# cgranerob/Land-Surface-Temperature-Super-Resolution-with-a-Scale-Invariance-Free-Neural-Approach

Measured on AMD Instinct MI355X. Metric: LST+NDVI 256x256 patches/sec (train fwd+bwd), whole job, higher is better.
Workload: dtype f32; 1 GPU; ModelB SIF-NN-SR2 (gradFTM loss) batch 64/GPU, synthetic 256x256, 1x MI355X, fwd+loss+bwd+Adam; batch_per_gpu=64, patch=256x256 (LST 64x64 + NDVI 256x256), parallelism=dp1, loss=sr2

## Files before the change

include/sifsr_hip.h:

```cpp
#ifndef SIFSR_HIP_H
#define SIFSR_HIP_H
#include <stddef.h>

#ifdef __cplusplus
#define SIFSR_API extern "C" __attribute__((visibility("default")))
#else
#define SIFSR_API
#endif

SIFSR_API int sifsr_abi_version(void);
SIFSR_API int sifsr_num_params(void);
SIFSR_API int sifsr_num_running(void);
SIFSR_API int sifsr_layer_table(int* out, int capacity_rows);

SIFSR_API size_t sifsr_model_workspace_bytes(int B, int H, int W, int training);
SIFSR_API int sifsr_model_workspace_regions(int B, int H, int W, size_t* out, int capacity);
SIFSR_API int sifsr_model_forward(const float* x, float* sr, const float* params, float* running, long long* nbt,
                                  void* workspace, size_t workspace_bytes, int B, int H, int W, int training,
                                  float momentum, float eps, void* stream);
SIFSR_API int sifsr_model_backward(const float* x, const float* dsr, const float* params, float* grads,
                                   void* workspace, size_t workspace_bytes, int B, int H, int W, void* stream);
SIFSR_API int sifsr_model_forward_ex(const float* x, float* sr, const float* params, float* running, long long* nbt,
                                     void* workspace, size_t workspace_bytes, int B, int H, int W, int training,
                                     float momentum, float eps, int compute, void* stream);
SIFSR_API int sifsr_model_backward_ex(const float* x, const float* dsr, const float* params, float* grads, void* workspace,
                                      size_t workspace_bytes, int B, int H, int W, int compute, void* stream);

SIFSR_API int sifsr_pack_conv_weights(const float* w_oihw, int cin, int cout, float* wfwd, float* wdgrad, void* stream);
SIFSR_API int sifsr_conv3x3_stat_blocks(int B, int H, int W, int cout);
SIFSR_API int sifsr_conv3x3_fwd(const float* src0, int C0, const float* scale0, const float* shift0,
                                const float* src1, int C1, const float* scale1, const float* shift1,
                                const float* wfwd, float* y, int cout, float* stat_partials, int B, int H, int W,
                                void* stream);
SIFSR_API int sifsr_conv3x3_dgrad(const float* dy, int cout, const float* wdgrad, const float* w_oihw, int cin,
                                  float* g0, int C0, float* g1, int C1, const float* addend, int B, int H, int W,
                                  void* stream);
SIFSR_API int sifsr_conv3x3_dgrad_fused(const float* g, const float* y, const float* coef_f, int cout, const float* wdgrad,
                                        const float* wwd, int cin, float* g0, int C0, float* g1, int C1, const float* addend,
                                        float* border, int B, int H, int W, void* stream);
SIFSR_API int sifsr_pack_conv_weights_wino(const float* w_oihw, int cin, int cout, float* wwf, float* wwd, void* stream);
SIFSR_API int sifsr_conv3x3_stat_blocks_wino(int B, int H, int W, int cin, int cout);
SIFSR_API int sifsr_conv3x3_fwd_wino(const float* src0, int C0, const float* scale0, const float* shift0,
                                     const float* src1, int C1, const float* scale1, const float* shift1,
                                     const float* wfwd, const float* wwf, float* y, int cout, float* stat_partials,
                                     int B, int H, int W, void* stream);
SIFSR_API int sifsr_conv3x3_dgrad_wino(const float* dy, int cout, const float* wdgrad, const float* wwd, int cin,
                                       float* g0, int C0, float* g1, int C1, const float* addend, int B, int H, int W,
                                       void* stream);
SIFSR_API int sifsr_conv3x3_fwd_bf16(const float* src0, int C0, const float* scale0, const float* shift0, const float* src1,
                                     int C1, const float* scale1, const float* shift1, const float* wdgrad, float* y,
                                     int cout, float* stat_partials, int B, int H, int W, void* stream);
SIFSR_API int sifsr_conv3x3_dgrad_bf16(const float* dy, int cout, const float* wdgrad, int cin, float* g0, int C0, float* g1,
                                       int C1, const float* addend, int B, int H, int W, void* stream);
SIFSR_API size_t sifsr_conv3x3_wgrad_scratch_floats(int cin, int cout, int nblk);
SIFSR_API int sifsr_conv3x3_wgrad(const float* src0, int C0, const float* scale0, const float* shift0,
                                  const float* src1, int C1, const float* scale1, const float* shift1,
                                  const float* dy, int cout, float* scratch, int nblk, float* dw, int B, int H, int W,
                                  void* stream);
SIFSR_API int sifsr_conv3x3_wgrad_fused(const float* src0, int C0, const float* scale0, const float* shift0,
                                        const float* src1, int C1, const float* scale1, const float* shift1,
                                        const float* g, const float* y, const float* coef_f, int cout, float* scratch,
                                        int nblk, float* dw, int B, int H, int W, void* stream);
// ... 118 lines not shown
```

land-surface-temperature-super-resolution-with-a-scale-invariance-free-neural-approach_amd/csrc/capi.hip:

```cpp
#include "../../include/sifsr_hip.h"

#include "engine.h"

#define S(stream) ((hipStream_t)(stream))

static ConvSrc mk_src(const float* p, int C, const float* sc, const float* sh) {
  ConvSrc s; s.ptr = p; s.scale = p ? sc : nullptr; s.shift = p ? sh : nullptr; s.C = p ? C : 0; s.coff = 0; s.nq = p ? C / 16 : 0;
  return s;
}

int sifsr_abi_version(void) { return 3; }
int sifsr_num_params(void) { return sifsr_net().total_params; }
int sifsr_num_running(void) { return sifsr_net().total_running; }
int sifsr_layer_table(int* out, int capacity_rows) {
  const NetTable& nt = sifsr_net();
  for (int l = 0; l < SIFSR_NUM_BN_LAYERS && l < capacity_rows; ++l) {
    const LayerInfo& L = nt.L[l];
    int* r = out + 8 * l;
    r[0] = L.cin; r[1] = L.cout; r[2] = L.level; r[3] = L.w_off; r[4] = L.gamma_off; r[5] = L.beta_off; r[6] = L.run_off; r[7] = L.ch_off;
  }
  return SIFSR_NUM_BN_LAYERS;
}

size_t sifsr_model_workspace_bytes(int B, int H, int W, int training) {
// ... 114 lines not shown
  int rc = launch_conv3x3_mfma(a, cin, 1, S(stream));
  if (rc) return rc;
  return launch_dgrad_border_fix(dy, cout, wdgrad, cin, g0, C0, C0, g1 ? g1 : g0, g1 ? C1 : C0, B, H, W, S(stream));
}

int sifsr_conv3x3_dgrad_fused(const float* g, const float* y, const float* coef_f, int cout, const float* wdgrad,
                              const float* wwd, int cin, float* g0, int C0, float* g1, int C1, const float* addend, float* border,
                              int B, int H, int W, void* stream) {
  if (cout % 16 || cin % 16 || C0 % 16 || (g1 && (C1 % 16 || C0 + C1 != cin)) || (!g1 && C0 != cin) || (addend && g1))
    return SIFSR_ERR_SHAPE;
  if (!g || !y || !coef_f || !border) return SIFSR_ERR_ARG;
  ConvArgs a;
  a.src[0] = mk_src(g, cout, nullptr, nullptr); a.src[1] = mk_src(nullptr, 0, nullptr, nullptr);
  a.bw_y = y; a.bw_coef = coef_f; a.bw_border = border;
  a.dst[0].ptr = g0; a.dst[0].C = C0; a.dst[0].coff = 0;
  a.dst[1].ptr = g1 ? g1 : g0; a.dst[1].C = g1 ? C1 : C0; a.dst[1].coff = 0;
  a.wpack = wdgrad; a.wpack_wino = wwd; a.addend = addend; a.addC = cin; a.stat_partials = nullptr; a.dst_split = C0 / 16;
  a.B = B; a.H = H; a.W = W; a.NQ = cout / 16;
  int rc = launch_conv3x3_mfma(a, cin, 1, S(stream));
  if (rc) return rc;
  return launch_dgrad_border_fix(border, cout, wdgrad, cin, g0, C0, C0, g1 ? g1 : g0, g1 ? C1 : C0, B, H, W, S(stream));
}

static int conv3x3_fwd_lowp(int mode, const float* src0, int C0, const float* scale0, const float* shift0, const float* src1, int C1,
                            const float* scale1, const float* shift1, const float* wdgrad, float* y, int cout,
                            float* stat_partials, int B, int H, int W, void* stream) {
  if (!src0 || !wdgrad || C0 % 16 || (src1 && C1 % 16)) return SIFSR_ERR_SHAPE;
  ConvArgs a;
  a.src[0] = mk_src(src0, C0, scale0, shift0);
  a.src[1] = mk_src(src1, C1, scale1, shift1);
  a.dst[0].ptr = y; a.dst[0].C = cout; a.dst[0].coff = 0; a.dst[1] = a.dst[0];
  a.NQ = a.src[0].nq + a.src[1].nq;
  const size_t n = (size_t)9 * (16 * a.NQ) * cout;
  a.wpack = wdgrad + n; a.bf16 = mode;
  a.addend = nullptr; a.addC = 0; a.stat_partials = stat_partials; a.dst_split = cout / 16;
  a.B = B; a.H = H; a.W = W;
  return launch_conv3x3_mfma(a, cout, 0, S(stream));
}
int sifsr_conv3x3_fwd_bf16(const float* src0, int C0, const float* scale0, const float* shift0, const float* src1, int C1,
                           const float* scale1, const float* shift1, const float* wdgrad, float* y, int cout,
                           float* stat_partials, int B, int H, int W, void* stream) {
  return conv3x3_fwd_lowp(1, src0, C0, scale0, shift0, src1, C1, scale1, shift1, wdgrad, y, cout, stat_partials, B, H, W, stream);
}
static int conv3x3_dgrad_lowp(int mode, const float* dy, int cout, const float* wdgrad, int cin, float* g0, int C0, float* g1, int C1,
                              const float* addend, int B, int H, int W, void* stream) {
  if (cout % 16 || cin % 16 || C0 % 16 || (g1 && (C1 % 16 || C0 + C1 != cin)) || (!g1 && C0 != cin) || (addend && g1))
// ... 372 lines not shown
```

land-surface-temperature-super-resolution-with-a-scale-invariance-free-neural-approach_amd/csrc/conv.h:

```cpp
#pragma once
#include "common.h"
#include "diag.h"

struct ConvSrc {
  const float* ptr;
  const float* scale;
  const float* shift;
  int C;
  int coff;
  int nq;
};

struct ConvDst {
  float* ptr;
  int C;
  int coff;
};

struct ConvArgs {
  ConvSrc src[2];
  ConvDst dst[2];
  const float* wpack;
  const float* wpack_wino = nullptr;
  const float* addend;
  float* stat_partials;
  int addC;
  int dst_split;
  int B, H, W;
  int NQ;
  int bf16 = 0;
  const float* bn_y = nullptr;
  const float* bn_scale = nullptr;
  const float* bn_shift = nullptr;
  const float* bw_y = nullptr;
  const float* bw_coef = nullptr;
  float* bw_border = nullptr;
};

int launch_conv3x3_mfma(const ConvArgs& a, int cout, int zero_pad, hipStream_t s);
bool conv3x3_use_wino(const ConvArgs& a, int cout);
bool conv3x3_wino8_applies(int nb, int nq);
int launch_conv3x3_wino8(const ConvArgs& a, int nb, int zero_pad, bool dyf, int grid, int ntiles, int lgx, int lgy, hipStream_t s);
int conv3x3_wino_kind(const ConvArgs& a, int cout, int zero_pad);
int conv3x3_grid_blocks(int B, int H, int W, int cout, int wino = 0);

struct WgradArgs {
  ConvSrc src[2];
  const float* dy;
  float* slabs;
  int B, H, W;
  int NQ;
  int ntiles;
  int bf16 = 0;
  const float* dy_y = nullptr;
  const float* dy_coef = nullptr;
};
int launch_conv3x3_wgrad(const WgradArgs& a, int cin, int cout, int nblk, hipStream_t s);
int wgrad_nbi_chunk(const WgradArgs& a, int cin);
int launch_wgrad_reduce(const float* slabs, int nblk, int cin, int cout, int nbi_chunk, float* dw_oihw, hipStream_t s);
size_t wgrad_slab_floats(int cin, int cout);
struct WgradReduceJob { size_t slab_off; int nblk, cin, cout, nbi_chunk, w_off; };
int launch_wgrad_reduce_batched(const float* ws, const WgradReduceJob* jobs, int njobs, float* grads, hipStream_t s);

bool conv3x3_wgrad_use_wino(const WgradArgs& a, int cin, int cout);
int wgrad_wino_nbi_chunk(int cin);
int launch_conv3x3_wgrad_wino(const WgradArgs& a, int cin, int cout, int nblk, hipStream_t s);
template <typename V4, typename GET>
// ... 26 lines not shown
  float* dy_border = nullptr;
  const float* wpack_wino;
  float* gin;
  const float* addend = nullptr;
  const float* bn_y = nullptr;
  const float* bn_scale = nullptr;
  const float* bn_shift = nullptr;
  float* stat_partials = nullptr;
  float* slabs;
  int B, H, W;
  const float* pool_gp = nullptr;
  int store_dz = 0;
  int half = 0;
};
bool conv3x3_bwd16_applies(int B, int H, int W);
int conv3x3_bwd16_grid(int B, int H, int W);
int launch_conv3x3_bwd16(const Bwd16Args& a, hipStream_t s);

int launch_dgrad_border_fix(const float* dy, int Cout, const float* wdg_layer, int Cin, float* g0, int C0,
                            int split_ch, float* g1, int C1, int B, int H, int W, hipStream_t s, int bf16 = 0,
                            const float* bn_y = nullptr, const float* bn_scale = nullptr, const float* bn_shift = nullptr,
                            float* bn_partials = nullptr, int masked = 0);
int dgrad_border_waves(int B, int H, int W, int Cin);

int launch_pack_weights(const float* params, float* wfwd, float* wdgrad, hipStream_t s, float* wwf = nullptr, float* wwd = nullptr,
                        long long* nbt = nullptr, int nbt_n = 0);
```

land-surface-temperature-super-resolution-with-a-scale-invariance-free-neural-approach_amd/csrc/conv_mfma.hip:

```cpp
#include "conv.h"

#include "switches.h"

namespace {

constexpr int PW = 18;
constexpr int PLANE = 336;
constexpr int WPITCH = 20, WHALF = 10, WPLANE = 364;

typedef __attribute__((ext_vector_type(4))) unsigned u32x4;

static __device__ __forceinline__ __amdgpu_buffer_rsrc_t make_rsrc(const float* p, unsigned bytes) {
  return __builtin_amdgcn_make_buffer_rsrc(const_cast<float*>(p), 0, (int)bytes, 0x00020000);
}
static __device__ __forceinline__ float4 bload4(__amdgpu_buffer_rsrc_t r, unsigned voff, unsigned soff) {
  const u32x4 v = __builtin_amdgcn_raw_buffer_load_b128(r, (int)voff, (int)soff, 0);
  return make_float4(__uint_as_float(v.x), __uint_as_float(v.y), __uint_as_float(v.z), __uint_as_float(v.w));
}
static __device__ __forceinline__ void bstore4(__amdgpu_buffer_rsrc_t r, unsigned voff, unsigned soff, float4 v) {
  u32x4 u;
  u.x = __float_as_uint(v.x); u.y = __float_as_uint(v.y); u.z = __float_as_uint(v.z); u.w = __float_as_uint(v.w);
  __builtin_amdgcn_raw_buffer_store_b128(u, r, (int)voff, (int)soff, 0);
}
constexpr unsigned OOB = 0xFFFFFF00u;
// ... 752 lines not shown
    if (corner) {
#pragma unroll
      for (int sd = 0; sd < 2; ++sd) {
        const int xc = sd == 0 ? 0 : W - 1;
        const bool on = (sd == 0 ? cl : cr) && valid && qx == xc;
        rv[0] = dyload(poff(qy, xc, on), (unsigned)q * 64u);
        rv[1] = dyload(poff(yin, xc, on), (unsigned)q * 64u);
        wv[0] = ld4(wbase + ((size_t)q * 9 + (8 - (1 * 3 + 2 * sd))) * 256);
        wv[1] = ld4(wbase + ((size_t)q * 9 + (8 - ((ty_tb + 1) * 3 + 2 * sd))) * 256);
        if (bf16) { rv[0] = round_bf16x4(rv[0]); rv[1] = round_bf16x4(rv[1]); }
        mac(wv[0], rv[0], false);
        mac(wv[1], add4(rv[0], rv[1]), false);
      }
    }
  }
  if (valid && !masked) {
    float4 v = g_old;
    v.x += acc[0]; v.y += acc[1]; v.z += acc[2]; v.w += acc[3];
    if (bf16) stA4<true>(dbase, de, v); else stA4<false>(dbase, de, v);
  }
  if (bn_partials != nullptr) {
    float d1[4] = {0.f, 0.f, 0.f, 0.f}, d2[4] = {0.f, 0.f, 0.f, 0.f};
    if (valid) {
      const float4 yv = bf16 ? ldA4<true>(bn_y, pix_o * 16 + 4 * kq) : ldA4<false>(bn_y, pix_o * 16 + 4 * kq);
      const float4 bsc = ld4(bn_scale + 4 * kq), bsh = ld4(bn_shift + 4 * kq);
      const float yy[4] = {yv.x, yv.y, yv.z, yv.w}, scv[4] = {bsc.x, bsc.y, bsc.z, bsc.w}, shv[4] = {bsh.x, bsh.y, bsh.z, bsh.w};
#pragma unroll
      for (int r = 0; r < 4; ++r) {
        const float dz = fmaf(yy[r], scv[r], shv[r]) > 0.f ? acc[r] : 0.f;
        d1[r] = dz; d2[r] = dz * yy[r];
      }
      if (masked) {
        const float4 v = make_float4(g_old.x + d1[0], g_old.y + d1[1], g_old.z + d1[2], g_old.w + d1[3]);
        if (bf16) stA4<true>(dbase, de, v); else stA4<false>(dbase, de, v);
      }
    }
#pragma unroll
    for (int r = 0; r < 4; ++r)
#pragma unroll
      for (int m = 1; m < 16; m <<= 1) { d1[r] += __shfl_xor(d1[r], m); d2[r] += __shfl_xor(d2[r], m); }
    if (px == 0) {
#pragma unroll
      for (int r = 0; r < 4; ++r) {
        bn_partials[((size_t)wave_g * 16 + 4 * kq + r) * 2 + 0] = d1[r];
        bn_partials[((size_t)wave_g * 16 + 4 * kq + r) * 2 + 1] = d2[r];
      }
    }
  }
}

}

bool conv3x3_use_wino(const ConvArgs& a, int cout) {
  return !sifsr_switches().no_wino && a.wpack_wino != nullptr && a.bf16 == 0 && cout <= 64 && a.H % 2 == 0 && a.W % 2 == 0 && (cout > 16 || a.NQ <= 2);
}

int conv3x3_wino_kind(const ConvArgs& a, int cout, int zero_pad) {
  if (!conv3x3_use_wino(a, cout)) return 0;
  return (cout == 16 && !zero_pad) ? 2 : 1;
}

int conv3x3_grid_blocks(int B, int H, int W, int cout, int wino) {
  const int ntiles = B * ((H + 15) / 16) * ((W + 15) / 16);
  const int per_cu = wino ? (wino == 2 ? 2 : 1) : (cout >= 64 ? 1 : 2);
  const int gmax = 256 * per_cu;
  if (ntiles <= gmax) return ntiles;
  const int rounds = (ntiles + gmax - 1) / gmax;
  int g = (ntiles + rounds - 1) / rounds;
  g = (g + 7) & ~7;
  return g < ntiles ? g : ntiles;
}

int launch_conv3x3_mfma(const ConvArgs& a, int cout, int zero_pad, hipStream_t s) {
  if (a.H < 1 || a.W < 1 || cout % 16 || a.NQ < 1 || a.src[0].nq + a.src[1].nq != a.NQ) return SIFSR_ERR_SHAPE;
  if (a.bf16 < 0 || a.bf16 > 1) return SIFSR_ERR_ARG;
  if (!a.src[0].ptr || !a.dst[0].ptr || !a.wpack) return SIFSR_ERR_ARG;
  const int ntiles = a.B * ((a.H + 15) / 16) * ((a.W + 15) / 16);
  const dim3 grid(conv3x3_grid_blocks(a.B, a.H, a.W, cout)), block(512);
  const int nb = cout / 16;
  const size_t npix = (size_t)a.B * a.H * a.W;
  auto pow2 = [](int v) { return v > 0 && (v & (v - 1)) == 0; };
  auto lg = [](int v) { int l = 0; while ((1 << l) < v) ++l; return l; };
  int cmax = a.src[0].C > a.src[1].C ? a.src[0].C : a.src[1].C;
  cmax = cmax > a.dst[0].C ? cmax : a.dst[0].C;
  cmax = cmax > a.dst[1].C ? cmax : a.dst[1].C;
  if (npix * cmax * 4 >= ((size_t)1 << 32) - 4096) return SIFSR_ERR_SHAPE;
  if (!pow2(a.src[0].C) || (a.src[1].ptr && !pow2(a.src[1].C))) return SIFSR_ERR_SHAPE;
  const int tx_ = (a.W + 15) / 16, ty_ = (a.H + 15) / 16;
  const int lgx = (pow2(tx_) && pow2(ty_)) ? lg(tx_) : -1, lgy = lgx >= 0 ? lg(ty_) : -1;
  const bool dyf = a.bw_y != nullptr;
  if (dyf && (!zero_pad || !a.bw_coef || a.src[1].ptr || a.src[0].scale || a.src[0].coff)) return SIFSR_ERR_ARG;
  if (nb == 8 && conv3x3_use_wino(a, 64) && a.stat_partials == nullptr && a.dst_split % 4 == 0) {
    for (int h = 0; h < 2; ++h) {
      ConvArgs w = a;
      w.wpack_wino = a.wpack_wino + (size_t)h * 4 * a.NQ * 16 * 256;
      const bool first = 4 * h < a.dst_split;
      w.dst[0] = first ? a.dst[0] : a.dst[1];
      w.dst[0].coff += first ? 64 * h : 16 * (4 * h - a.dst_split);
      w.dst[1] = w.dst[0];
      w.dst_split = 4;
      if (a.addend != nullptr) w.addend = a.addend + 64 * h;
      const int rc = launch_conv3x3_mfma(w, 64, zero_pad, s);
      if (rc != SIFSR_OK) return rc;
    }
    return SIFSR_OK;
  }
  if (conv3x3_use_wino(a, cout)) {
    ConvArgs w = a;
    w.wpack = a.wpack_wino;
    const dim3 wgrid(conv3x3_grid_blocks(a.B, a.H, a.W, cout, conv3x3_wino_kind(a, cout, zero_pad)));
    if (conv3x3_wino8_applies(nb, a.NQ)) return launch_conv3x3_wino8(w, nb, zero_pad, dyf, (int)wgrid.x, ntiles, lgx, lgy, s);
#define SIFSR_WINO_LAUNCH(NBV, ZP, DY) hipLaunchKernelGGL((conv3x3_mfma_kernel<NBV, ZP, 0, DY, true>), wgrid, block, 0, s, w, ntiles, lgx, lgy)
#define SIFSR_WINO_CASE(NBV)                                                                              \
  case NBV:                                                                                               \
// ... 59 lines not shown
  SIFSR_LAUNCH_CHECK();
  return SIFSR_OK;
}

int launch_pack_weights_one(const float* w, int cin, int cout, float* wfwd, float* wdg, hipStream_t s, float* wwf, float* wwd) {
  PackTable tb;
  tb.w_off[0] = 0; tb.cin[0] = cin; tb.cout[0] = cout; tb.p_off[0] = 0;
  const int n = 9 * cin * cout;
  const dim3 grid((n + 255) / 256 > 64 ? 64 : (n + 255) / 256, 1);
  if (wfwd != nullptr && wdg != nullptr) {
    hipLaunchKernelGGL(pack_weights_kernel, grid, dim3(256), 0, s, w, wfwd, wdg, tb);
    SIFSR_LAUNCH_CHECK();
  }
  if (wwf != nullptr && wwd != nullptr) {
    hipLaunchKernelGGL(pack_wino_kernel, dim3(grid.x * 2, 1), dim3(256), 0, s, w, wwf, wwd, tb);
    SIFSR_LAUNCH_CHECK();
  }
  return SIFSR_OK;
}

int dgrad_border_waves(int B, int H, int W, int Cin) {
  return B * (2 * ((W + 15) / 16) + 2 * ((H - 2 + 15) / 16)) * (Cin / 16);
}

int launch_dgrad_border_fix(const float* dy, int Cout, const float* wdg_layer, int Cin, float* g0, int C0,
                            int split_ch, float* g1, int C1, int B, int H, int W, hipStream_t s, int bf16,
                            const float* bn_y, const float* bn_scale, const float* bn_shift, float* bn_partials, int masked) {
  if (bn_partials != nullptr && (Cin != 16 || !bn_y || !bn_scale || !bn_shift)) return SIFSR_ERR_ARG;
  if (masked && bn_partials == nullptr) return SIFSR_ERR_ARG;
  if (H < 3 || W < 2 || Cin % 16 || Cout % 16) return SIFSR_ERR_SHAPE;
  const int waves = B * (2 * ((W + 15) / 16) + 2 * ((H - 2 + 15) / 16)) * (Cin / 16);
  hipLaunchKernelGGL(dgrad_border_kernel, dim3((waves + 3) / 4), dim3(256), 0, s, dy, Cout, wdg_layer, Cin, g0, C0,
                     split_ch, g1, C1, B, H, W, bf16, bn_y, bn_scale, bn_shift, bn_partials, masked);
  SIFSR_LAUNCH_CHECK();
  return SIFSR_OK;
}
```

land-surface-temperature-super-resolution-with-a-scale-invariance-free-neural-approach_amd/csrc/conv_wino8.hip:

```cpp
#include "conv.h"
#include "switches.h"

SIFSR_DIAG_CLOCK_DECL
SIFSR_DIAG_CLOCK8_DECL
namespace {

constexpr int PW = 18;
constexpr int WPITCH = 20, WHALF = 10, WPLANE = 364;

typedef __attribute__((ext_vector_type(4))) unsigned u32x4;
static __device__ __forceinline__ __amdgpu_buffer_rsrc_t make_rsrc(const float* p, unsigned bytes) {
  return __builtin_amdgcn_make_buffer_rsrc(const_cast<float*>(p), 0, (int)bytes, 0x00020000);
}
static __device__ __forceinline__ float4 bload4(__amdgpu_buffer_rsrc_t r, unsigned voff, unsigned soff) {
  const u32x4 v = __builtin_amdgcn_raw_buffer_load_b128(r, (int)voff, (int)soff, 0);
  return make_float4(__uint_as_float(v.x), __uint_as_float(v.y), __uint_as_float(v.z), __uint_as_float(v.w));
}
static __device__ __forceinline__ void bstore4(__amdgpu_buffer_rsrc_t r, unsigned voff, unsigned soff, float4 v) {
  u32x4 u;
  u.x = __float_as_uint(v.x); u.y = __float_as_uint(v.y); u.z = __float_as_uint(v.z); u.w = __float_as_uint(v.w);
  __builtin_amdgcn_raw_buffer_store_b128(u, r, (int)voff, (int)soff, 0);
}
constexpr unsigned OOB = 0xFFFFFF00u;

template <int NB, bool ZERO_PAD, bool DYF>
__global__ __launch_bounds__(512, 2) void conv3x3_wino8_kernel(const ConvArgs a, const int ntiles, const int lgx, const int lgy) {
  static_assert(NB == 2 || NB == 4, "32 or 64 output channels");
  static_assert(!DYF || ZERO_PAD, "the fused BatchNorm backward belongs to the input-gradient pass");
  constexpr int NGRP = NB == 4 ? 2 : 1;

  __shared__ float4 lds[2][4 * WPLANE];
  __shared__ float red[8][16][2];
  __shared__ float4 coef[8][4][4];

  const int tid = threadIdx.x;
  const int lane = tid & 63;
  const int wave8 = __builtin_amdgcn_readfirstlane(tid >> 6);
  __builtin_amdgcn_s_setprio(2);
  const int H = a.H, W = a.W;
  const int tiles_x = (W + 15) / 16, tiles_y = (H + 15) / 16;
  const int NQ = a.NQ;
  const unsigned npix = (unsigned)a.B * (unsigned)H * (unsigned)W;

  const int G = gridDim.x;
  const bool xcd_map = (G % 8 == 0) && (ntiles % 8 == 0);
  const int t_lo = xcd_map ? (blockIdx.x % 8) * (ntiles / 8) : 0;
  const int t_hi = xcd_map ? t_lo + ntiles / 8 : ntiles;
  const int t_step = xcd_map ? G / 8 : G;
  int t = t_lo + (xcd_map ? blockIdx.x / 8 : blockIdx.x);
  auto tile_pos = [&](int tt, int& tb, int& txi, int& tyi) {
    if (lgx >= 0) { tyi = (tt >> lgx) & (tiles_y - 1); tb = tt >> (lgx + lgy); txi = (tt + tyi + tb) & (tiles_x - 1); }
    else { txi = tt % tiles_x; const int r = tt / tiles_x; tyi = r % tiles_y; tb = r / tiles_y; }
  };

  const __amdgpu_buffer_rsrc_t rs0 = make_rsrc(a.src[0].ptr, npix * a.src[0].C * 4u);
  const __amdgpu_buffer_rsrc_t rs1 = make_rsrc(a.src[1].ptr ? a.src[1].ptr : a.src[0].ptr, npix * (a.src[1].ptr ? a.src[1].C : a.src[0].C) * 4u);
// ... 51 lines not shown
    const int ch = (first ? a.src[0].coff + 16 * q : a.src[1].coff + 16 * (q - a.src[0].nq));
    const unsigned soff = ((unsigned)pix_base << lgc) + (unsigned)ch * 4u;
    const __amdgpu_buffer_rsrc_t r = first ? rs0 : rs1;
#pragma unroll
    for (int it = 0; it < 3; ++it) {
      const unsigned voff = (ZERO_PAD && pixv[it] < 0) ? OOB : (((unsigned)pixv[it] << lgc) + (unsigned)cg * 16u);
      stg[it] = bload4(r, voff, soff);
      if (DYF) sty[it] = bload4(rsy, voff, soff);
    }
    if (it_q + 1 < NQ) ++it_q;
    else if (it_t + t_step < t_hi) { it_t += t_step; it_q = 0; set_tile(it_t); }
  };
  if (tid < NQ * 16) {
    const int q = tid >> 4, kind = (tid >> 2) & 3, c4 = tid & 3;
    const bool first = q < a.src[0].nq;
    const int C = first ? a.src[0].C : a.src[1].C;
    const int ch = (first ? a.src[0].coff + 16 * q : a.src[1].coff + 16 * (q - a.src[0].nq));
    const float* scp = first ? a.src[0].scale : a.src[1].scale;
    const float* shp = first ? a.src[0].shift : a.src[1].shift;
    float4 v = make_float4(0.f, 0.f, 0.f, 0.f);
    if (DYF) v = ld4(a.bw_coef + kind * C + ch + 4 * c4);
    else if (scp != nullptr && kind < 2) v = ld4((kind ? shp : scp) + ch + 4 * c4);
    coef[q][kind][c4] = v;
  }
  auto write_stage = [&](float4* Lb) {
    const int q = stg_q, tS = stg_t;
    const bool first = q < a.src[0].nq;
    const bool praw = !DYF && (first ? a.src[0].scale : a.src[1].scale) == nullptr;
    const float4 psc = coef[q][0][cg], psh = coef[q][1][cg];
    float4 k1A = psc, k0A = psc;
    if (DYF) { k1A = coef[q][2][cg]; k0A = coef[q][3][cg]; }
    int wb = 0, wy0 = 0, wx0 = 0;
    bool winterior = true;
    if (DYF) {
      int txi, tyi;
      tile_pos(tS, wb, txi, tyi);
      wy0 = tyi * 16 - 1; wx0 = txi * 16 - 1;
      winterior = txi > 0 && tyi > 0 && txi + 1 < tiles_x && tyi + 1 < tiles_y;
    }
#pragma unroll
    for (int it = 0; it < 3; ++it) {
      float4 v = stg[it];
      const bool mine = it < 2 || st2;
      if (DYF) {
        v = bn_bwd4(v, sty[it], psc, psh, k1A, k0A);
        if (!winterior) {
// ... 130 lines not shown
        for (int b = 0; b < 4; ++b) Mc[b] = __builtin_amdgcn_mfma_f32_16x16x4f32(wr[b].w, dh[ar][b][1], Mc[b], 0, 0, 0);
        if (g == NGRP - 1) {
          __builtin_amdgcn_sched_barrier(0);
#pragma unroll
          for (int b = 0; b < 4; ++b) wq[4 * ar + b] = bload4(rww, (unsigned)lane * 16u, wsoff(qn, 4 * ar + b));
        }
        if (ar > 0) out_row(ar - 1, M[(ar - 1) & 1]);
      }
      out_row(3, M[1]);
      SIFSR_DIAG_T(g3_);
      SIFSR_DIAG_ADD(dt_rd, g1_ - g0_); SIFSR_DIAG_ADD(dt_tr, g2_ - g1_); SIFSR_DIAG_ADD(dt_mm, g3_ - g2_);
    }
    __builtin_amdgcn_s_setprio(3);
    SIFSR_DIAG_T(c2);

    if (!stage_first && more) {
      write_stage(lds[buf ^ 1]);
      issue_loads();
    }

    if (last_q) {
      int cb, txi, tyi;
      tile_pos(t, cb, txi, tyi);
      const bool do_stats = a.stat_partials != nullptr;
      const bool d0 = nb0 < a.dst_split;
      const int dC = d0 ? a.dst[0].C : a.dst[1].C;
      const __amdgpu_buffer_rsrc_t rd = d0 ? rd0 : rd1;
      const unsigned chb = (unsigned)((d0 ? a.dst[0].coff + 16 * nb0 : a.dst[1].coff + 16 * (nb0 - a.dst_split)) + 4 * kq) * 4u;
#pragma unroll
      for (int g = 0; g < NGRP; ++g) {
#pragma unroll
        for (int o = 0; o < 4; ++o) {
          const int oy = o >> 1, ox = o & 1;
          const int yy = tyi * 16 + g0 + 4 * g + 2 * pyl + oy, xx = txi * 16 + 2 * pxp + ox;
          const bool ok = yy < H && xx < W;
          f32x4 v = Y[g][oy][ox];
          Y[g][oy][ox] = zero4;
          const unsigned pixo = (unsigned)((cb * H + yy) * W + xx);
          if (a.addend != nullptr) {
            const float4 ad = bload4(rad, ok ? pixo * (unsigned)a.addC * 4u + (unsigned)(16 * nb0 + 4 * kq) * 4u : OOB, 0u);
            v[0] += ad.x; v[1] += ad.y; v[2] += ad.z; v[3] += ad.w;
          }
          bstore4(rd, ok ? pixo * (unsigned)dC * 4u + chb : OOB, 0u, make_float4(v[0], v[1], v[2], v[3]));
          if (do_stats) {
            if (!ok) v = zero4;
#pragma unroll
            for (int r = 0; r < 4; ++r) { s1[r] += v[r]; s2[r] = fmaf(v[r], v[r], s2[r]); }
          }
        }
      }
    }
    SIFSR_DIAG_T(c3);
    __syncthreads();
    SIFSR_DIAG_T(c4);
    SIFSR_DIAG_ACC8(0, (c1 - c0) + (c3 - c2)); SIFSR_DIAG_ACC8(1, dt_rd); SIFSR_DIAG_ACC8(2, dt_tr); SIFSR_DIAG_ACC8(3, dt_mm);
    SIFSR_DIAG_ACC8(4, c4 - c3); SIFSR_DIAG_ACC8(5, 1);
    buf ^= 1;
    if (last_q) { t = t_next; q = 0; } else ++q;
  };
  for (int j = 0; j < n_items; ++j) do_item(j);

  SIFSR_DIAG_CLOCK_END(tid)
  SIFSR_DIAG_ACC8_FLUSH(wave8 >= 4 ? 6 : 0)
  if (a.stat_partials != nullptr) {
    const int px = lane & 15;
#pragma unroll
    for (int r = 0; r < 4; ++r) {
      float u = s1[r], v = s2[r];
#pragma unroll
      for (int m = 1; m < 16; m <<= 1) { u += __shfl_xor(u, m); v += __shfl_xor(v, m); }
      if (px == 0) { red[wave8][4 * kq + r][0] = u; red[wave8][4 * kq + r][1] = v; }
    }
    __syncthreads();
    if (tid < NB * 16) {
      const int nb = tid >> 4, cc = tid & 15;
      float u = 0.f, v = 0.f;
      for (int w = nb; w < 8; w += NB) { u += red[w][cc][0]; v += red[w][cc][1]; }
      float* o = a.stat_partials + ((size_t)blockIdx.x * (NB * 16) + tid) * 2;
      o[0] = u; o[1] = v;
    }
  }
}

}

bool conv3x3_wino8_applies(int nb, int nq) {
  return !sifsr_switches().no_wino8 && (nb == 2 || nb == 4) && nq <= 8;
}

int launch_conv3x3_wino8(const ConvArgs& a, int nb, int zero_pad, bool dyf, int grid, int ntiles, int lgx, int lgy, hipStream_t s) {
  const dim3 g(grid), block(512);
#define SIFSR_W8L(NBV)                                                                                                            \
  {                                                                                                                               \
    if (dyf) hipLaunchKernelGGL((conv3x3_wino8_kernel<NBV, true, true>),     g, block, 0, s, a, ntiles, lgx, lgy);               \
    else if (zero_pad) hipLaunchKernelGGL((conv3x3_wino8_kernel<NBV, true, false>),     g, block, 0, s, a, ntiles, lgx, lgy);    \
    else hipLaunchKernelGGL((conv3x3_wino8_kernel<NBV, false, false>),     g, block, 0, s, a, ntiles, lgx, lgy);                 \
    SIFSR_LAUNCH_CHECK();                                                                                                         \
// ... 10 lines not shown
```

land-surface-temperature-super-resolution-with-a-scale-invariance-free-neural-approach_amd/csrc/engine.hip:

```cpp
#include "engine.h"
#include "switches.h"

#include <stdio.h>
#include <stdlib.h>

#include <mutex>
#include <vector>

static thread_local bool t_half_storage = false;
bool sifsr_half_storage() { return t_half_storage; }
HalfStorageScope::HalfStorageScope(bool on) : prev(t_half_storage) { t_half_storage = on; }
HalfStorageScope::~HalfStorageScope() { t_half_storage = prev; }

static int env_int(const char* name, int dflt) { const char* v = getenv(name); return v ? atoi(v) : dflt; }
const Switches& sifsr_switches() {
  static const Switches sw = {
      env_int("SIFSR_WGRAD_STREAM", 1), env_int("SIFSR_WGRAD_WINO", 2),  env_int("SIFSR_NO_WINO", 0),
      env_int("SIFSR_NO_WINO8", 0),     env_int("SIFSR_NO_BWD16", 0),    env_int("SIFSR_TAIL_APPLY", 0),
      env_int("SIFSR_HEAD_LINEAR", 0),  env_int("SIFSR_BF16_BWD16", 0),  env_int("SIFSR_DBG_EARLY_REDUCE", 3),
      env_int("SIFSR_DBG_POOL_ON_LOAD", 1)};
  return sw;
}

static constexpr int enc_prev[3] = {L_IN3, L_D1C, L_D2C};
// ... 60 lines not shown
    w.P[k] = take(pc[k] * N[k + 1]);
    w.R[k] = take(pc[k] * N[k + 1]);
  }
  for (int k = 0; k < 3; ++k) w.U[k] = take(uc[k] * N[2 - k]);

  size_t maxpart = 0;
  for (int l = 0; l < SIFSR_NUM_BN_LAYERS; ++l) {
    const int lh = H >> nt.L[l].level, lw = W >> nt.L[l].level;
    const size_t nblk = (size_t)B * ((lh + 15) / 16) * ((lw + 15) / 16);
    const size_t n = (nblk > 1024 ? nblk : 1024) * nt.L[l].cout * 2;
    maxpart = n > maxpart ? n : maxpart;
  }
  for (int k = 0; k < 3; ++k) {
    const int lh = H >> (3 - k), lw = W >> (3 - k);
    const size_t n = (size_t)up2x_bwd_stat_rows(B, lh, lw, uc[k]) * uc[k] * 2;
    maxpart = n > maxpart ? n : maxpart;
  }
  w.partials = take(maxpart);
  w.partials_cap = maxpart;
  w.fwd_end = off;
  if (training) {
    w.coef = take(6 * 64);
    w.coef_f = take(4 * (size_t)nt.total_channels);
    w.bpart = take((size_t)dgrad_border_waves(B, H, W, 16) * 32);
    for (int l = 0; l < SIFSR_NUM_BN_LAYERS; ++l) w.g[l] = take(nt.L[l].cout * N[nt.L[l].level]);
    w.dy_border = take(16 * N[0]);
    w.dyB[0] = w.dyB[1] = w.dyB[2] = w.dy_border;
    for (int k = 0; k < 3; ++k) w.gP[k] = take(pc[k] * N[k + 1]);
    for (int k = 0; k < 3; ++k) w.gU[k] = take(uc[k] * N[2 - k]);
    w.slabs = take(1024 * 288);
    w.gram = take(conv_in_gram_scratch_floats());
    w.slab_l[0] = 0; w.slab_cap[0] = 0;
    for (int l = 1; l < SIFSR_NUM_BN_LAYERS; ++l) {
      const int lvh = H >> nt.L[l].level, lvw = W >> nt.L[l].level;
      const int ntiles = B * ((lvh + 7) / 8) * ((lvw + 15) / 16);
      const int nb_tap = wgrad_blocks(nt.L[l].cin, nt.L[l].cout, 1, ntiles, false), nb_wino = wgrad_blocks(nt.L[l].cin, nt.L[l].cout, 1, ntiles, true);
      w.slab_cap[l] = (size_t)(nb_tap > nb_wino ? nb_tap : nb_wino) * 9 * nt.L[l].cin * nt.L[l].cout;
      if (nt.L[l].cin == 16 && nt.L[l].cout == 16 && conv3x3_bwd16_applies(B, lvh, lvw)) {
        const size_t need = (size_t)conv3x3_bwd16_grid(B, lvh, lvw) * 9 * 256;
        if (need > w.slab_cap[l]) w.slab_cap[l] = need;
      }
      w.slab_l[l] = take(w.slab_cap[l]);
    }
  }
  w.total = off;
  return SIFSR_OK;
}
// ... 158 lines not shown
  a.B = c.B; a.H = c.lvH(L.level); a.W = c.lvW(L.level);
  a.NQ = L.cin / 16;
  {
    ProfScope ps(l, 1, c.s);
    SIFSR_TRY(launch_conv3x3_mfma(a, L.cout, 0, c.s));
  }
  if (training)
    SIFSR_TRY(bn_unit_finalize(c, l, conv3x3_grid_blocks(c.B, a.H, a.W, L.cout, conv3x3_wino_kind(a, L.cout, 0)), running, momentum, eps));
  return SIFSR_OK;
}

int bn_bwd_reduce_blocks(size_t npix) {
  const size_t nb = npix / 256;
  return (int)(nb > 1024 ? 1024 : (nb < 1 ? 1 : nb));
}
int bn_unit_bwd(const Ctx& c, int l, const float* gp = nullptr, int fused_stats = 0, int border_rows = -1,
                bool writeback = true) {
  const LayerInfo& L = c.nt.L[l];
  const int lh = c.lvH(L.level), lw = c.lvW(L.level);
  const size_t npix = c.lay.npix[L.level];
  float* dgamma = c.grads + L.gamma_off, *dbeta = c.grads + L.beta_off;
  if (fused_stats > 0) {
    if (gp != nullptr) return SIFSR_ERR_ARG;
    return launch_bn_bwd_finalize2(c.f(c.lay.partials), fused_stats, c.f(c.lay.bpart), border_rows >= 0 ? border_rows : dgrad_border_waves(c.B, lh, lw, 16),
                                   L.cout, (double)npix, c.scale(l), c.mean(l), c.invstd(l), dgamma, dbeta, c.coef(), c.s, c.shift(l),
                                   c.params + L.beta_off, c.coef_f(l));
  }
  const int nblk = bn_bwd_reduce_blocks(npix);
  SIFSR_TRY(launch_bn_bwd_reduce(c.g(l), c.y(l), c.scale(l), c.shift(l), c.mean(l), c.invstd(l), L.cout, npix, c.f(c.lay.partials), nblk,
                                 c.s, gp, lh, lw, (gp && writeback) ? c.g(l) : nullptr));
  return launch_bn_bwd_finalize(c.f(c.lay.partials), nblk, L.cout, (double)npix, c.scale(l), c.mean(l), c.invstd(l), dgamma, dbeta,
                                c.coef(), c.s, c.shift(l), c.params + L.beta_off, c.coef_f(l));
}

static bool wgrad_wino_policy(int cout) {
  const int mode = sifsr_switches().wgrad_wino;
  return mode == 2 || (mode == 1 && cout <= 32);
}

int conv_unit_wgrad(const Ctx& c, int l, ConvSrc s0, ConvSrc s1, const float* dy, bool dy_stored = false) {
  const LayerInfo& L = c.nt.L[l];
  WgradArgs a;
  a.src[0] = s0; a.src[1] = s1;
  a.dy = dy; a.slabs = c.slab(l);
  if (!dy_stored) { a.dy_y = c.y(l); a.dy_coef = c.coef_f(l); }
  a.B = c.B; a.H = c.lvH(L.level); a.W = c.lvW(L.level);
  a.NQ = L.cin / 16;
// ... 3 lines not shown
  const int nbi = wino ? wgrad_wino_nbi_chunk(L.cin) : wgrad_nbi_chunk(a, L.cin);
  const int nblk = wgrad_blocks(L.cin, L.cout, L.cin / (16 * nbi), a.ntiles, wino);
  if ((size_t)nblk * (L.cin / (16 * nbi)) * 9 * (16 * nbi) * L.cout > c.lay.slab_cap[l]) return SIFSR_ERR_WORKSPACE;
  hipStream_t ws = c.s;
  if (c.side != nullptr) {
    if (hipEventRecord(c.side->ev[l], c.s) != hipSuccess || hipStreamWaitEvent(c.side->s, c.side->ev[l], 0) != hipSuccess)
      return SIFSR_ERR_ARG;
    ws = c.side->s;
    *c.forked = true;
  }
  {
    ProfScope ps(l, 3, ws);
    if (wino) SIFSR_TRY(launch_conv3x3_wgrad_wino(a, L.cin, L.cout, nblk, ws));
    else SIFSR_TRY(launch_conv3x3_wgrad(a, L.cin, L.cout, nblk, ws));
  }
  WgradReduceJob& j = c.bwd->jobs[c.bwd->njobs++];
  j.slab_off = c.lay.slab_l[l]; j.nblk = nblk; j.cin = L.cin; j.cout = L.cout; j.nbi_chunk = nbi; j.w_off = L.w_off;
  return SIFSR_OK;
}

int conv_unit_dgrad(const Ctx& c, int l, const float* dy, float* g0, int C0, int split_ch, float* g1, int C1,
                    const float* addend, int bn_layer = -1, int* stat_rows = nullptr, bool dy_stored = false) {
  const LayerInfo& L = c.nt.L[l];
  const bool fuse = bn_layer >= 0 && L.cin == 16 && C0 == 16 && split_ch == 16 && g1 == nullptr && addend == nullptr &&
                    c.nt.L[bn_layer].cout == 16 && c.nt.L[bn_layer].level == L.level;
  if (stat_rows) *stat_rows = 0;
  ConvArgs a;
  a.src[0] = src_raw(dy, L.cout); a.src[1] = src_none();
  const float* dy_edge = dy;
  if (!dy_stored) {
    a.bw_y = c.y(l); a.bw_coef = c.coef_f(l); a.bw_border = c.f(c.lay.dy_border);
    dy_edge = a.bw_border;
  }
  a.dst[0].ptr = g0; a.dst[0].C = C0; a.dst[0].coff = 0;
  a.dst[1].ptr = g1 ? g1 : g0; a.dst[1].C = g1 ? C1 : C0; a.dst[1].coff = 0;
  a.bf16 = c.bf16;
  a.wpack = c.w_dgrad(l);
  a.wpack_wino = c.w_dgrad_wino(l);
  a.addend = addend; a.addC = L.cin;
  a.stat_partials = nullptr;
  a.dst_split = split_ch / 16;
  a.B = c.B; a.H = c.lvH(L.level); a.W = c.lvW(L.level);
  a.NQ = L.cout / 16;
  if (fuse) {
    a.stat_partials = c.f(c.lay.partials);
    a.bn_y = c.y(bn_layer); a.bn_scale = c.scale(bn_layer); a.bn_shift = c.shift(bn_layer);
    if (stat_rows) *stat_rows = conv3x3_grid_blocks(c.B, a.H, a.W, L.cin, conv3x3_wino_kind(a, L.cin, 1));
  }
  {
    ProfScope ps(l, 2, c.s);
    SIFSR_TRY(launch_conv3x3_mfma(a, L.cin, 1, c.s));
  }
  SIFSR_TRY(launch_dgrad_border_fix(dy_edge, L.cout, c.w_dgrad_f32(l), L.cin, g0, C0, split_ch, g1 ? g1 : g0, g1 ? C1 : C0, c.B, a.H,
                                    a.W, c.s, c.bf16, fuse ? a.bn_y : nullptr, fuse ? a.bn_scale : nullptr,
                                    fuse ? a.bn_shift : nullptr, fuse ? c.f(c.lay.bpart) : nullptr));
  return SIFSR_OK;
}

bool bwd16_usable(const Ctx& c, int l, ConvSrc s0) {
  const LayerInfo& L = c.nt.L[l];
  return L.cin == 16 && L.cout == 16 && (c.bf16 == 0 || sifsr_switches().bf16_bwd16) && wgrad_wino_policy(16) && s0.C == 16 &&
         s0.coff == 0 && conv3x3_bwd16_applies(c.B, c.lvH(L.level), c.lvW(L.level));
}
int conv_unit_bwd16(const Ctx& c, int l, ConvSrc s0, const float* dy, float* gin, const float* addend, int bn_layer, int* stat_rows,
                    int dy_mode, bool* applied, bool store_dz = false, const float* pool_gp = nullptr) {
  const LayerInfo& L = c.nt.L[l];
  *applied = false;
  if (stat_rows) *stat_rows = 0;
  const int lh = c.lvH(L.level), lw = c.lvW(L.level);
  if (!bwd16_usable(c, l, s0)) return dy_mode == 2 ? SIFSR_ERR_ARG : SIFSR_OK;
// ... 271 lines not shown
```

Before: 10740 patches/s.

## Fuse BN-backward statistics into wino8 dgrad for 32/64-channel layers

Extends the fused dgrad+BN-backward-statistics path, previously limited to 16-channel layers, to 32- and 64-channel layers that use the Winograd-8 dgrad kernel. The kernel now reads the BN output y, applies the ReLU mask, and accumulates dgamma/dbeta partials per channel. The border-fix kernel is generalised to handle any Cin for those partials, and its workspace is sized per layer. This removes a separate BN-backward reduction pass over the gradient tensor, in exchange for extra loads and register pressure in the dgrad epilogue. It also adds a C API entry point for the fused path.

```diff
diff --git a/include/sifsr_hip.h b/include/sifsr_hip.h
--- a/include/sifsr_hip.h
+++ b/include/sifsr_hip.h
@@ -38,6 +38,17 @@
 SIFSR_API int sifsr_conv3x3_dgrad_fused(const float* g, const float* y, const float* coef_f, int cout, const float* wdgrad,
                                         const float* wwd, int cin, float* g0, int C0, float* g1, int C1, const float* addend,
                                         float* border, int B, int H, int W, void* stream);
+typedef struct SifsrDgradBnArgs {
+  const float* g; const float* y; const float* coef_f; int cout;
+  const float* wdgrad; const float* wwd; int cin;
+  float* gin; float* border;
+  const float* bn_y; const float* bn_scale; const float* bn_shift;
+  float* stat_partials; float* border_partials;
+  int B, H, W;
+} SifsrDgradBnArgs;
+SIFSR_API int sifsr_conv3x3_stat_rows_dgrad_bn(int B, int H, int W, int cin, int cout, int has_wwd);
+SIFSR_API int sifsr_conv3x3_stat_rows_dgrad_border(int B, int H, int W);
+SIFSR_API int sifsr_conv3x3_dgrad_fused_bn(const SifsrDgradBnArgs* args, void* stream);
 SIFSR_API int sifsr_pack_conv_weights_wino(const float* w_oihw, int cin, int cout, float* wwf, float* wwd, void* stream);
 SIFSR_API int sifsr_conv3x3_stat_blocks_wino(int B, int H, int W, int cin, int cout);
 SIFSR_API int sifsr_conv3x3_fwd_wino(const float* src0, int C0, const float* scale0, const float* shift0,
diff --git a/land-surface-temperature-super-resolution-with-a-scale-invariance-free-neural-approach_amd/csrc/capi.hip b/land-surface-temperature-super-resolution-with-a-scale-invariance-free-neural-approach_amd/csrc/capi.hip
--- a/land-surface-temperature-super-resolution-with-a-scale-invariance-free-neural-approach_amd/csrc/capi.hip
+++ b/land-surface-temperature-super-resolution-with-a-scale-invariance-free-neural-approach_amd/csrc/capi.hip
@@ -160,6 +160,39 @@
   return launch_dgrad_border_fix(border, cout, wdgrad, cin, g0, C0, C0, g1 ? g1 : g0, g1 ? C1 : C0, B, H, W, S(stream));
 }
 
+static ConvArgs dgrad_bn_args(const SifsrDgradBnArgs& p) {
+  ConvArgs a;
+  a.src[0] = mk_src(p.g, p.cout, nullptr, nullptr); a.src[1] = mk_src(nullptr, 0, nullptr, nullptr);
+  a.bw_y = p.y; a.bw_coef = p.coef_f; a.bw_border = p.border;
+  a.dst[0].ptr = p.gin; a.dst[0].C = p.cin; a.dst[0].coff = 0; a.dst[1] = a.dst[0];
+  a.wpack = p.wdgrad; a.wpack_wino = p.wwd; a.addend = nullptr; a.addC = p.cin; a.dst_split = p.cin / 16;
+  a.stat_partials = p.stat_partials; a.bn_y = p.bn_y; a.bn_scale = p.bn_scale; a.bn_shift = p.bn_shift;
+  a.B = p.B; a.H = p.H; a.W = p.W; a.NQ = p.cout / 16;
+  return a;
+}
+int sifsr_conv3x3_stat_rows_dgrad_bn(int B, int H, int W, int cin, int cout, int has_wwd) {
+  if (B < 1 || H < 1 || W < 1 || cin < 16 || cin % 16 || cout < 16 || cout % 16) return 0;
+  SifsrDgradBnArgs p = {};
+  p.cin = cin; p.cout = cout; p.B = B; p.H = H; p.W = W;
+  p.y = reinterpret_cast<const float*>(1);
+  p.wwd = has_wwd ? reinterpret_cast<const float*>(1) : nullptr;
+  return conv3x3_dgrad_bn_rows(dgrad_bn_args(p), cin);
+}
+int sifsr_conv3x3_stat_rows_dgrad_border(int B, int H, int W) { return dgrad_border_rows(B, H, W); }
+int sifsr_conv3x3_dgrad_fused_bn(const SifsrDgradBnArgs* args, void* stream) {
+  if (!args) return SIFSR_ERR_ARG;
+  const SifsrDgradBnArgs& p = *args;
+  if (p.cout < 16 || p.cout % 16 || p.cin < 16 || p.cin % 16) return SIFSR_ERR_SHAPE;
+  if (!p.g || !p.y || !p.coef_f || !p.border || !p.wdgrad || !p.gin || !p.bn_y || !p.bn_scale || !p.bn_shift || !p.stat_partials ||
+      !p.border_partials)
+    return SIFSR_ERR_ARG;
+  const ConvArgs a = dgrad_bn_args(p);
+  int rc = launch_conv3x3_mfma(a, p.cin, 1, S(stream));
+  if (rc) return rc;
+  return launch_dgrad_border_fix(p.border, p.cout, p.wdgrad, p.cin, p.gin, p.cin, p.cin, p.gin, p.cin, p.B, p.H, p.W, S(stream), 0,
+                                 p.bn_y, p.bn_scale, p.bn_shift, p.border_partials);
+}
+
 static int conv3x3_fwd_lowp(int mode, const float* src0, int C0, const float* scale0, const float* shift0, const float* src1, int C1,
                             const float* scale1, const float* shift1, const float* wdgrad, float* y, int cout,
                             float* stat_partials, int B, int H, int W, void* stream) {
diff --git a/land-surface-temperature-super-resolution-with-a-scale-invariance-free-neural-approach_amd/csrc/conv.h b/land-surface-temperature-super-resolution-with-a-scale-invariance-free-neural-approach_amd/csrc/conv.h
--- a/land-surface-temperature-super-resolution-with-a-scale-invariance-free-neural-approach_amd/csrc/conv.h
+++ b/land-surface-temperature-super-resolution-with-a-scale-invariance-free-neural-approach_amd/csrc/conv.h
@@ -43,6 +43,7 @@
 int launch_conv3x3_wino8(const ConvArgs& a, int nb, int zero_pad, bool dyf, int grid, int ntiles, int lgx, int lgy, hipStream_t s);
 int conv3x3_wino_kind(const ConvArgs& a, int cout, int zero_pad);
 int conv3x3_grid_blocks(int B, int H, int W, int cout, int wino = 0);
+int conv3x3_dgrad_bn_rows(const ConvArgs& a, int cin);
 
 struct WgradArgs {
   ConvSrc src[2];
@@ -115,6 +116,7 @@
                             const float* bn_y = nullptr, const float* bn_scale = nullptr, const float* bn_shift = nullptr,
                             float* bn_partials = nullptr, int masked = 0);
 int dgrad_border_waves(int B, int H, int W, int Cin);
+int dgrad_border_rows(int B, int H, int W);
 
 int launch_pack_weights(const float* params, float* wfwd, float* wdgrad, hipStream_t s, float* wwf = nullptr, float* wwd = nullptr,
                         long long* nbt = nullptr, int nbt_n = 0);
diff --git a/land-surface-temperature-super-resolution-with-a-scale-invariance-free-neural-approach_amd/csrc/conv_mfma.hip b/land-surface-temperature-super-resolution-with-a-scale-invariance-free-neural-approach_amd/csrc/conv_mfma.hip
--- a/land-surface-temperature-super-resolution-with-a-scale-invariance-free-neural-approach_amd/csrc/conv_mfma.hip
+++ b/land-surface-temperature-super-resolution-with-a-scale-invariance-free-neural-approach_amd/csrc/conv_mfma.hip
@@ -798,8 +798,8 @@
   if (bn_partials != nullptr) {
     float d1[4] = {0.f, 0.f, 0.f, 0.f}, d2[4] = {0.f, 0.f, 0.f, 0.f};
     if (valid) {
-      const float4 yv = bf16 ? ldA4<true>(bn_y, pix_o * 16 + 4 * kq) : ldA4<false>(bn_y, pix_o * 16 + 4 * kq);
-      const float4 bsc = ld4(bn_scale + 4 * kq), bsh = ld4(bn_shift + 4 * kq);
+      const float4 yv = bf16 ? ldA4<true>(bn_y, pix_o * Cin + ci_o) : ldA4<false>(bn_y, pix_o * Cin + ci_o);
+      const float4 bsc = ld4(bn_scale + ci_o), bsh = ld4(bn_shift + ci_o);
       const float yy[4] = {yv.x, yv.y, yv.z, yv.w}, scv[4] = {bsc.x, bsc.y, bsc.z, bsc.w}, shv[4] = {bsh.x, bsh.y, bsh.z, bsh.w};
 #pragma unroll
       for (int r = 0; r < 4; ++r) {
@@ -816,11 +816,9 @@
 #pragma unroll
       for (int m = 1; m < 16; m <<= 1) { d1[r] += __shfl_xor(d1[r], m); d2[r] += __shfl_xor(d2[r], m); }
     if (px == 0) {
-#pragma unroll
-      for (int r = 0; r < 4; ++r) {
-        bn_partials[((size_t)wave_g * 16 + 4 * kq + r) * 2 + 0] = d1[r];
-        bn_partials[((size_t)wave_g * 16 + 4 * kq + r) * 2 + 1] = d2[r];
-      }
+      float* o = bn_partials + ((size_t)(wave_g / NBI) * Cin + ci_o) * 2;
+#pragma unroll
+      for (int r = 0; r < 4; ++r) { o[2 * r + 0] = d1[r]; o[2 * r + 1] = d2[r]; }
     }
   }
 }
@@ -834,6 +832,15 @@
 int conv3x3_wino_kind(const ConvArgs& a, int cout, int zero_pad) {
   if (!conv3x3_use_wino(a, cout)) return 0;
   return (cout == 16 && !zero_pad) ? 2 : 1;
+}
+
+int conv3x3_dgrad_bn_rows(const ConvArgs& a, int cin) {
+  if (cin == 16) return conv3x3_grid_blocks(a.B, a.H, a.W, 16, conv3x3_wino_kind(a, 16, 1));
+  const int nb = cin / 16;
+  if ((cin != 32 && cin != 64) || a.bw_y == nullptr || a.addend != nullptr || a.dst_split != nb || a.dst[0].C != cin || a.dst[0].coff != 0)
+    return 0;
+  if (!conv3x3_use_wino(a, cin) || !conv3x3_wino8_applies(nb, a.NQ)) return 0;
+  return conv3x3_grid_blocks(a.B, a.H, a.W, cin, conv3x3_wino_kind(a, cin, 1));
 }
 
 int conv3x3_grid_blocks(int B, int H, int W, int cout, int wino) {
@@ -866,6 +873,9 @@
   const int lgx = (pow2(tx_) && pow2(ty_)) ? lg(tx_) : -1, lgy = lgx >= 0 ? lg(ty_) : -1;
   const bool dyf = a.bw_y != nullptr;
   if (dyf && (!zero_pad || !a.bw_coef || a.src[1].ptr || a.src[0].scale || a.src[0].coff)) return SIFSR_ERR_ARG;
+  if (a.bn_y != nullptr && (!zero_pad || !a.bn_scale || !a.bn_shift || !a.stat_partials || conv3x3_dgrad_bn_rows(a, cout) == 0))
+    return SIFSR_ERR_ARG;
+  if (zero_pad && a.stat_partials != nullptr && a.bn_y == nullptr) return SIFSR_ERR_ARG;
   if (nb == 8 && conv3x3_use_wino(a, 64) && a.stat_partials == nullptr && a.dst_split % 4 == 0) {
     for (int h = 0; h < 2; ++h) {
       ConvArgs w = a;
@@ -971,12 +981,13 @@
 int dgrad_border_waves(int B, int H, int W, int Cin) {
   return B * (2 * ((W + 15) / 16) + 2 * ((H - 2 + 15) / 16)) * (Cin / 16);
 }
+int dgrad_border_rows(int B, int H, int W) { return dgrad_border_waves(B, H, W, 16); }
 
 int launch_dgrad_border_fix(const float* dy, int Cout, const float* wdg_layer, int Cin, float* g0, int C0,
                             int split_ch, float* g1, int C1, int B, int H, int W, hipStream_t s, int bf16,
                             const float* bn_y, const float* bn_scale, const float* bn_shift, float* bn_partials, int masked) {
-  if (bn_partials != nullptr && (Cin != 16 || !bn_y || !bn_scale || !bn_shift)) return SIFSR_ERR_ARG;
-  if (masked && bn_partials == nullptr) return SIFSR_ERR_ARG;
+  if (bn_partials != nullptr && (!bn_y || !bn_scale || !bn_shift || split_ch != Cin || C0 != Cin)) return SIFSR_ERR_ARG;
+  if (masked && (bn_partials == nullptr || Cin != 16)) return SIFSR_ERR_ARG;
   if (H < 3 || W < 2 || Cin % 16 || Cout % 16) return SIFSR_ERR_SHAPE;
   const int waves = B * (2 * ((W + 15) / 16) + 2 * ((H - 2 + 15) / 16)) * (Cin / 16);
   hipLaunchKernelGGL(dgrad_border_kernel, dim3((waves + 3) / 4), dim3(256), 0, s, dy, Cout, wdg_layer, Cin, g0, C0,
diff --git a/land-surface-temperature-super-resolution-with-a-scale-invariance-free-neural-approach_amd/csrc/conv_wino8.hip b/land-surface-temperature-super-resolution-with-a-scale-invariance-free-neural-approach_amd/csrc/conv_wino8.hip
--- a/land-surface-temperature-super-resolution-with-a-scale-invariance-free-neural-approach_amd/csrc/conv_wino8.hip
+++ b/land-surface-temperature-super-resolution-with-a-scale-invariance-free-neural-approach_amd/csrc/conv_wino8.hip
@@ -32,6 +32,8 @@
   __shared__ float4 lds[2][4 * WPLANE];
   __shared__ float red[8][16][2];
   __shared__ float4 coef[8][4][4];
+  __shared__ float4 bnc[DYF ? 2 * NB * 4 : 1];
+  const bool bn_stats = DYF && a.stat_partials != nullptr;
 
   const int tid = threadIdx.x;
   const int lane = tid & 63;
@@ -129,6 +131,10 @@
     if (DYF) v = ld4(a.bw_coef + kind * C + ch + 4 * c4);
     else if (scp != nullptr && kind < 2) v = ld4((kind ? shp : scp) + ch + 4 * c4);
     coef[q][kind][c4] = v;
+  }
+  if (DYF && bn_stats && tid < 2 * NB * 4) {
+    const int kind = tid / (NB * 4), c4 = tid % (NB * 4);
+    bnc[tid] = ld4((kind ? a.bn_shift : a.bn_scale) + 4 * c4);
   }
   auto write_stage = [&](float4* Lb) {
     const int q = stg_q, tS = stg_t;
@@ -305,11 +311,14 @@
     if (last_q) {
       int cb, txi, tyi;
       tile_pos(t, cb, txi, tyi);
-      const bool do_stats = a.stat_partials != nullptr;
+      const bool do_stats = !DYF && a.stat_partials != nullptr;
       const bool d0 = nb0 < a.dst_split;
       const int dC = d0 ? a.dst[0].C : a.dst[1].C;
       const __amdgpu_buffer_rsrc_t rd = d0 ? rd0 : rd1;
       const unsigned chb = (unsigned)((d0 ? a.dst[0].coff + 16 * nb0 : a.dst[1].coff + 16 * (nb0 - a.dst_split)) + 4 * kq) * 4u;
+      const __amdgpu_buffer_rsrc_t rby = make_rsrc(bn_stats ? a.bn_y : a.dst[0].ptr, npix * (unsigned)(NB * 16) * 4u);
+      float4 bsc = make_float4(0.f, 0.f, 0.f, 0.f), bsh = bsc;
+      if (DYF && bn_stats) { bsc = bnc[4 * nb0 + kq]; bsh = bnc[NB * 4 + 4 * nb0 + kq]; }
 #pragma unroll
       for (int g = 0; g < NGRP; ++g) {
 #pragma unroll
@@ -324,8 +333,18 @@
             const float4 ad = bload4(rad, ok ? pixo * (unsigned)a.addC * 4u + (unsigned)(16 * nb0 + 4 * kq) * 4u : OOB, 0u);
             v[0] += ad.x; v[1] += ad.y; v[2] += ad.z; v[3] += ad.w;
           }
-          bstore4(rd, ok ? pixo * (unsigned)dC * 4u + chb : OOB, 0u, make_float4(v[0], v[1], v[2], v[3]));
-          if (do_stats) {
+          const unsigned voff = ok ? pixo * (unsigned)dC * 4u + chb : OOB;
+          bstore4(rd, voff, 0u, make_float4(v[0], v[1], v[2], v[3]));
+          if (DYF && bn_stats) {
+            const float4 yv = bload4(rby, voff, 0u);
+            const float yy4[4] = {yv.x, yv.y, yv.z, yv.w};
+            const float scv[4] = {bsc.x, bsc.y, bsc.z, bsc.w}, shv[4] = {bsh.x, bsh.y, bsh.z, bsh.w};
+#pragma unroll
+            for (int r = 0; r < 4; ++r) {
+              const float dz = (ok && fmaf(yy4[r], scv[r], shv[r]) > 0.f) ? v[r] : 0.f;
+              s1[r] += dz; s2[r] = fmaf(dz, yy4[r], s2[r]);
+            }
+          } else if (do_stats) {
             if (!ok) v = zero4;
 #pragma unroll
             for (int r = 0; r < 4; ++r) { s1[r] += v[r]; s2[r] = fmaf(v[r], v[r], s2[r]); }
@@ -346,16 +365,19 @@
   SIFSR_DIAG_CLOCK_END(tid)
   SIFSR_DIAG_ACC8_FLUSH(wave8 >= 4 ? 6 : 0)
   if (a.stat_partials != nullptr) {
-    const int px = lane & 15;
+    const int lane_e = DYF ? (int)__builtin_amdgcn_mbcnt_hi(~0u, __builtin_amdgcn_mbcnt_lo(~0u, 0u)) : lane;
+    const int tid_e = DYF ? wave8 * 64 + lane_e : tid;
+    const int px = lane_e & 15, kq_e = lane_e >> 4;
 #pragma unroll
     for (int r = 0; r < 4; ++r) {
       float u = s1[r], v = s2[r];
 #pragma unroll
       for (int m = 1; m < 16; m <<= 1) { u += __shfl_xor(u, m); v += __shfl_xor(v, m); }
-      if (px == 0) { red[wave8][4 * kq + r][0] = u; red[wave8][4 * kq + r][1] = v; }
+      if (px == 0) { red[wave8][4 * kq_e + r][0] = u; red[wave8][4 * kq_e + r][1] = v; }
     }
     __syncthreads();
-    if (tid < NB * 16) {
+    if (tid_e < NB * 16) {
+      const int tid = tid_e;
       const int nb = tid >> 4, cc = tid & 15;
       float u = 0.f, v = 0.f;
       for (int w = nb; w < 8; w += NB) { u += red[w][cc][0]; v += red[w][cc][1]; }
diff --git a/land-surface-temperature-super-resolution-with-a-scale-invariance-free-neural-approach_amd/csrc/engine.hip b/land-surface-temperature-super-resolution-with-a-scale-invariance-free-neural-approach_amd/csrc/engine.hip
--- a/land-surface-temperature-super-resolution-with-a-scale-invariance-free-neural-approach_amd/csrc/engine.hip
+++ b/land-surface-temperature-super-resolution-with-a-scale-invariance-free-neural-approach_amd/csrc/engine.hip
@@ -106,7 +106,13 @@
   if (training) {
     w.coef = take(6 * 64);
     w.coef_f = take(4 * (size_t)nt.total_channels);
-    w.bpart = take((size_t)dgrad_border_waves(B, H, W, 16) * 32);
+    size_t bpart = 0;
+    for (int l = 0; l < SIFSR_NUM_BN_LAYERS; ++l) {
+      if (nt.L[l].cout > 64) continue;
+      const size_t n = (size_t)dgrad_border_waves(B, H >> nt.L[l].level, W >> nt.L[l].level, nt.L[l].cout) * 32;
+      bpart = n > bpart ? n : bpart;
+    }
+    w.bpart = take(bpart);
     for (int l = 0; l < SIFSR_NUM_BN_LAYERS; ++l) w.g[l] = take(nt.L[l].cout * N[nt.L[l].level]);
     w.dy_border = take(16 * N[0]);
     w.dyB[0] = w.dyB[1] = w.dyB[2] = w.dy_border;
@@ -311,7 +317,7 @@
   float* dgamma = c.grads + L.gamma_off, *dbeta = c.grads + L.beta_off;
   if (fused_stats > 0) {
     if (gp != nullptr) return SIFSR_ERR_ARG;
-    return launch_bn_bwd_finalize2(c.f(c.lay.partials), fused_stats, c.f(c.lay.bpart), border_rows >= 0 ? border_rows : dgrad_border_waves(c.B, lh, lw, 16),
+    return launch_bn_bwd_finalize2(c.f(c.lay.partials), fused_stats, c.f(c.lay.bpart), border_rows >= 0 ? border_rows : dgrad_border_rows(c.B, lh, lw),
                                    L.cout, (double)npix, c.scale(l), c.mean(l), c.invstd(l), dgamma, dbeta, c.coef(), c.s, c.shift(l),
                                    c.params + L.beta_off, c.coef_f(l));
   }
@@ -361,8 +367,8 @@
 int conv_unit_dgrad(const Ctx& c, int l, const float* dy, float* g0, int C0, int split_ch, float* g1, int C1,
                     const float* addend, int bn_layer = -1, int* stat_rows = nullptr, bool dy_stored = false) {
   const LayerInfo& L = c.nt.L[l];
-  const bool fuse = bn_layer >= 0 && L.cin == 16 && C0 == 16 && split_ch == 16 && g1 == nullptr && addend == nullptr &&
-                    c.nt.L[bn_layer].cout == 16 && c.nt.L[bn_layer].level == L.level;
+  const bool fusable = bn_layer >= 0 && C0 == L.cin && split_ch == L.cin && g1 == nullptr && addend == nullptr &&
+                       c.nt.L[bn_layer].cout == L.cin && c.nt.L[bn_layer].level == L.level;
   if (stat_rows) *stat_rows = 0;
   ConvArgs a;
   a.src[0] = src_raw(dy, L.cout); a.src[1] = src_none();
@@ -381,10 +387,13 @@
   a.dst_split = split_ch / 16;
   a.B = c.B; a.H = c.lvH(L.level); a.W = c.lvW(L.level);
   a.NQ = L.cout / 16;
+  int rows = fusable ? conv3x3_dgrad_bn_rows(a, L.cin) : 0;
+  if ((size_t)rows * L.cin * 2 > c.lay.partials_cap) rows = 0;
+  const bool fuse = rows > 0;
   if (fuse) {
     a.stat_partials = c.f(c.lay.partials);
     a.bn_y = c.y(bn_layer); a.bn_scale = c.scale(bn_layer); a.bn_shift = c.shift(bn_layer);
-    if (stat_rows) *stat_rows = conv3x3_grid_blocks(c.B, a.H, a.W, L.cin, conv3x3_wino_kind(a, L.cin, 1));
+    if (stat_rows) *stat_rows = rows;
   }
   {
     ProfScope ps(l, 2, c.s);
```

After: 10580 patches/s. 0.986x the previous value.
